# chanchanchan97/ICAFusion

Measured on AMD Instinct MI355X. Metric: RGB/IR image-pairs/sec (two-stream forward + NMS), higher is better.
Workload: dtype bf16

## Files before the change

### icafusion_amd/csrc/pool.hip

```cpp
#include "icaf_common.h"
#include <cstdlib>
#include <algorithm>
#include <cstdint>

namespace icaf {

template <int DT>
__global__ __launch_bounds__(256) void preprocess_kernel(const float* __restrict__ img, typename Elem<DT>::type* __restrict__ out,
                                                         int B, int C, int H, int W, int Cpad, int mode) {
    using E = Elem<DT>;
    const int Ho = mode ? H / 2 : H, Wo = mode ? W / 2 : W;
    const long long npix = (long long)B * Ho * Wo;
    const int nv = Cpad / E::VEC;
    for (long long pix = (long long)blockIdx.x * blockDim.x + threadIdx.x; pix < npix; pix += (long long)gridDim.x * blockDim.x) {
        const int wo = (int)(pix % Wo);
        const long long t = pix / Wo;
        const int ho = (int)(t % Ho), b = (int)(t / Ho);
        for (int v = 0; v < nv; ++v) {
            float f[E::VEC];
#pragma unroll
            for (int j = 0; j < E::VEC; ++j) {
                const int ch = v * E::VEC + j;
                float val = 0.0f;
                if (mode == 0) {
                    if (ch < C) val = img[(((long long)b * C + ch) * H + ho) * W + wo];
                } else if (ch < 4 * C) {
                    const int sub = ch / C, c = ch - sub * C, dy = sub >> 1, dx = sub & 1;
                    val = img[(((long long)b * C + c) * H + 2 * ho + dy) * W + 2 * wo + dx];
                }
                f[j] = val;
            }
            *(u32x4*)(out + pix * Cpad + v * E::VEC) = pack16<DT>(f);
        }
    }
}

template <int DT>
__global__ __launch_bounds__(256) void preprocess_u8_kernel(const unsigned char* __restrict__ img, typename Elem<DT>::type* __restrict__ out,
                                                            int B, int Ctot, int c0, int C, int nstreams, int H, int W, int Cpad, int mode) {
    using E = Elem<DT>;
    const int Ho = mode ? H / 2 : H, Wo = mode ? W / 2 : W;
    const long long npix = (long long)nstreams * B * Ho * Wo;
    const int nv = Cpad / E::VEC;
    for (long long pix = (long long)blockIdx.x * blockDim.x + threadIdx.x; pix < npix; pix += (long long)gridDim.x * blockDim.x) {
        const int wo = (int)(pix % Wo);
        long long t = pix / Wo;
        const int ho = (int)(t % Ho);
        t /= Ho;
        const int b = (int)(t % B), st = (int)(t / B);
        const unsigned char* src = img + ((long long)b * Ctot + c0 + st * C) * H * W;
        for (int v = 0; v < nv; ++v) {
            float f[E::VEC];
#pragma unroll
            for (int j = 0; j < E::VEC; ++j) {
                const int ch = v * E::VEC + j;
                float val = 0.0f;
                if (mode == 0) {
                    if (ch < C) val = (float)src[((long long)ch * H + ho) * W + wo] / 255.0f;
                } else if (ch < 4 * C) {
                    const int sub = ch / C, c = ch - sub * C, dy = sub >> 1, dx = sub & 1;
                    val = (float)src[((long long)c * H + 2 * ho + dy) * W + 2 * wo + dx] / 255.0f;
                }
                f[j] = val;
            }
            *(u32x4*)(out + pix * Cpad + v * E::VEC) = pack16<DT>(f);
        }
    }
}


template <int DT>
__global__ __launch_bounds__(256) void sppf_kernel(const typename Elem<DT>::type* __restrict__ x, int ldx,
                                                   typename Elem<DT>::type* __restrict__ y1, typename Elem<DT>::type* __restrict__ y2,
                                                   typename Elem<DT>::type* __restrict__ y3, int ldy, int B, int H, int W, int C, int k) {
    using E = Elem<DT>;
    const int nv = C / E::VEC;
    const long long total = (long long)B * H * W * nv;
    const int r1 = k / 2, r2 = 2 * r1, r3 = 3 * r1;
    for (long long idx = (long long)blockIdx.x * blockDim.x + threadIdx.x; idx < total; idx += (long long)gridDim.x * blockDim.x) {
        const int v = (int)(idx % nv);
        const long long pix = idx / nv;
        const int w = (int)(pix % W);
        const long long t = pix / W;
        const int h = (int)(t % H), b = (int)(t / H);
        float m1[E::VEC], m2[E::VEC], m3[E::VEC];
#pragma unroll
        for (int j = 0; j < E::VEC; ++j) m1[j] = m2[j] = m3[j] = -INFINITY;
        for (int dy = -r3; dy <= r3; ++dy) {
            const int hh = h + dy;
            if ((unsigned)hh >= (unsigned)H) continue;
            const int ady = dy < 0 ? -dy : dy;
            for (int dx = -r3; dx <= r3; ++dx) {
                const int ww = w + dx;
                if ((unsigned)ww >= (unsigned)W) continue;
                const int adx = dx < 0 ? -dx : dx;
                const int rad = ady > adx ? ady : adx;
                float f[E::VEC];
                unpack16<DT>(*(const u32x4*)(x + (((long long)b * H + hh) * W + ww) * ldx + v * E::VEC), f);
#pragma unroll
                for (int j = 0; j < E::VEC; ++j) {
                    m3[j] = fmaxf(m3[j], f[j]);
                    if (rad <= r2) m2[j] = fmaxf(m2[j], f[j]);
                    if (rad <= r1) m1[j] = fmaxf(m1[j], f[j]);
                }
            }
        }
        const long long o = pix * ldy + v * E::VEC;
        *(u32x4*)(y1 + o) = pack16<DT>(m1);
        *(u32x4*)(y2 + o) = pack16<DT>(m2);
        *(u32x4*)(y3 + o) = pack16<DT>(m3);
    }
}


__device__ __forceinline__ unsigned int key16x2(unsigned int b) {
    const unsigned int sign = b & 0x80008000u;
    return b ^ ((sign >> 15) * 0x7fffu | 0x80008000u);
}
__device__ __forceinline__ u32x4 key_vec(u32x4 v) { return u32x4{key16x2(v[0]), key16x2(v[1]), key16x2(v[2]), key16x2(v[3])}; }
__device__ __forceinline__ unsigned int unkey16x2(unsigned int k) {
    const unsigned int pos = k & 0x80008000u;
    return k ^ (((pos ^ 0x80008000u) >> 15) * 0x7fffu | 0x80008000u);
}
__device__ __forceinline__ u32x4 unkey_vec(u32x4 v) { return u32x4{unkey16x2(v[0]), unkey16x2(v[1]), unkey16x2(v[2]), unkey16x2(v[3])}; }
__device__ __forceinline__ unsigned int max_u16x2(unsigned int a, unsigned int b) {
    using u16x2 = __attribute__((ext_vector_type(2))) unsigned short;
    const u16x2 x = __builtin_bit_cast(u16x2, a), y = __builtin_bit_cast(u16x2, b);
    const u16x2 m = __builtin_elementwise_max(x, y);
    return __builtin_bit_cast(unsigned int, m);
}

template <int DT> struct PlaneMax {
    static __device__ __forceinline__ u32x4 in(u32x4 v) { return key_vec(v); }
    static __device__ __forceinline__ u32x4 out(u32x4 v) { return unkey_vec(v); }
    static __device__ __forceinline__ u32x4 mx(u32x4 a, u32x4 b) {
        return u32x4{max_u16x2(a[0], b[0]), max_u16x2(a[1], b[1]), max_u16x2(a[2], b[2]), max_u16x2(a[3], b[3])};
    }
};
template <> struct PlaneMax<ICAF_F32> {
    static __device__ __forceinline__ u32x4 in(u32x4 v) { return v; }
    static __device__ __forceinline__ u32x4 out(u32x4 v) { return v; }
    static __device__ __forceinline__ u32x4 mx(u32x4 a, u32x4 b) {
        u32x4 r;
#pragma unroll
        for (int j = 0; j < 4; ++j) r[j] = __float_as_uint(fmaxf(__uint_as_float(a[j]), __uint_as_float(b[j])));
        return r;
    }
};

template <int DT>
__global__ __launch_bounds__(256) void sppf_lds_kernel(const typename Elem<DT>::type* __restrict__ x, int ldx,
                                                       typename Elem<DT>::type* __restrict__ y1, typename Elem<DT>::type* __restrict__ y2,
                                                       typename Elem<DT>::type* __restrict__ y3, int ldy, int H, int W, int C, int k,
                                                       int vpb) {
    using E = Elem<DT>;
    using PM = PlaneMax<DT>;
    extern __shared__ __attribute__((aligned(16))) unsigned char smem[];
    u32x4* cur = (u32x4*)smem;
    u32x4* tmp = cur + (size_t)H * W * vpb;
    const int nvb = (C / E::VEC) / vpb;
    const int b = blockIdx.x / nvb, vg = blockIdx.x - b * nvb;
    const int n = H * W * vpb, r = k / 2;
    const long long pix0 = (long long)b * H * W;
    constexpr int MAXIT = 8;
    short iv[MAXIT], ix[MAXIT], iy[MAXIT];
#pragma unroll
    for (int t = 0; t < MAXIT; ++t) {
        const int i = threadIdx.x + t * 256;
        const int ii = i < n ? i : 0;
        const int v = ii % vpb, pp = ii / vpb;
        iv[t] = (short)v; ix[t] = (short)(pp % W); iy[t] = (short)(pp / W);
    }
#pragma unroll
    for (int t = 0; t < MAXIT; ++t) {
        const int i = threadIdx.x + t * 256;
        if (i < n) cur[i] = PM::in(*(const u32x4*)(x + (pix0 + iy[t] * W + ix[t]) * ldx + (vg * vpb + iv[t]) * E::VEC));
    }
    __syncthreads();
    typename E::type* outs[3] = {y1, y2, y3};
#pragma unroll
    for (int stage = 0; stage < 3; ++stage) {
#pragma unroll
        for (int t = 0; t < MAXIT; ++t) {
            const int i = threadIdx.x + t * 256;
            if (i >= n) continue;
            const int xx = ix[t];
            u32x4 m = cur[i];
            for (int d = -r; d <= r; ++d) {
                if (d == 0 || (unsigned)(xx + d) >= (unsigned)W) continue;
                m = PM::mx(m, cur[i + d * vpb]);
            }
            tmp[i] = m;
        }
        __syncthreads();
#pragma unroll
        for (int t = 0; t < MAXIT; ++t) {
            const int i = threadIdx.x + t * 256;
            if (i >= n) continue;
            const int yy = iy[t];
            u32x4 m = tmp[i];
            for (int d = -r; d <= r; ++d) {
                if (d == 0 || (unsigned)(yy + d) >= (unsigned)H) continue;
                m = PM::mx(m, tmp[i + d * W * vpb]);
            }
            cur[i] = m;
            *(u32x4*)(outs[stage] + (pix0 + yy * W + ix[t]) * ldy + (vg * vpb + iv[t]) * E::VEC) = PM::out(m);
        }
        __syncthreads();
    }
}

struct PoolDiv { FastDiv nv, wo, ho; };

template <int DT, bool I32>
__global__ __launch_bounds__(256) void maxpool_kernel(const typename Elem<DT>::type* __restrict__ x, int ldx, typename Elem<DT>::type* __restrict__ y,
                                                      int ldy, int B, int H, int W, int Ho, int Wo, int nv, int k, int st, int pad, PoolDiv dv) {
    using E = Elem<DT>;
    const long long total = (long long)B * Ho * Wo * nv;
    for (long long idx = (long long)blockIdx.x * blockDim.x + threadIdx.x; idx < total; idx += (long long)gridDim.x * blockDim.x) {
        long long pix;
        int v, wo, ho, b;
        if constexpr (I32) {
            unsigned int upix, uv, t, uwo, ub, uho;
            fd_divmod((unsigned int)idx, dv.nv, upix, uv);
            fd_divmod(upix, dv.wo, t, uwo);
            fd_divmod(t, dv.ho, ub, uho);
            pix = upix; v = (int)uv; wo = (int)uwo; ho = (int)uho; b = (int)ub;
        } else {
            v = (int)(idx % nv);
            pix = idx / nv;
            wo = (int)(pix % Wo);
            const long long t = pix / Wo;
            ho = (int)(t % Ho);
            b = (int)(t / Ho);
        }
        float m[E::VEC];
#pragma unroll
        for (int j = 0; j < E::VEC; ++j) m[j] = -INFINITY;
        const int h0 = ho * st - pad, w0 = wo * st - pad;
        for (int dy = 0; dy < k; ++dy) {
            const int hh = h0 + dy;
            if ((unsigned)hh >= (unsigned)H) continue;
            for (int dx = 0; dx < k; ++dx) {
                const int ww = w0 + dx;
                if ((unsigned)ww >= (unsigned)W) continue;
                float f[E::VEC];
                unpack16<DT>(*(const u32x4*)(x + (((long long)b * H + hh) * W + ww) * ldx + v * E::VEC), f);
#pragma unroll
                for (int j = 0; j < E::VEC; ++j) m[j] = (f[j] > m[j] || f[j] != f[j]) ? f[j] : m[j];
            }
        }
        *(u32x4*)(y + pix * ldy + v * E::VEC) = pack16<DT>(m);
    }
}

template <int DT>
__global__ __launch_bounds__(256) void maxpool_scalar_kernel(const typename Elem<DT>::type* __restrict__ x, int ldx, typename Elem<DT>::type* __restrict__ y,
                                                             int ldy, int B, int H, int W, int Ho, int Wo, int C, int k, int st, int pad) {
    using E = Elem<DT>;
    const long long total = (long long)B * Ho * Wo * C;
    for (long long idx = (long long)blockIdx.x * blockDim.x + threadIdx.x; idx < total; idx += (long long)gridDim.x * blockDim.x) {
        const int c = (int)(idx % C);
        const long long pix = idx / C;
        const int wo = (int)(pix % Wo);
        const long long t = pix / Wo;
        const int ho = (int)(t % Ho), b = (int)(t / Ho);
        float m = -INFINITY;
        const int h0 = ho * st - pad, w0 = wo * st - pad;
        for (int dy = 0; dy < k; ++dy) {
            const int hh = h0 + dy;
            if ((unsigned)hh >= (unsigned)H) continue;
            for (int dx = 0; dx < k; ++dx) {
                const int ww = w0 + dx;
                if ((unsigned)ww >= (unsigned)W) continue;
                const float f = E::ld(x + (((long long)b * H + hh) * W + ww) * ldx + c);
                m = (f > m || f != f) ? f : m;
            }
        }
        E::st(y + pix * ldy + c, m);
    }
}

struct UpsampleDiv { FastDiv nv, wo, ho, scale; };

template <bool I32>
__global__ __launch_bounds__(256) void upsample_kernel(const u32x4* __restrict__ x, int ldxv, u32x4* __restrict__ y, int ldyv,
                                                       int B, int H, int W, int nv, int scale, UpsampleDiv dv) {
    const int Ho = H * scale, Wo = W * scale;
    const long long total = (long long)B * Ho * Wo * nv;
    for (long long idx = (long long)blockIdx.x * blockDim.x + threadIdx.x; idx < total; idx += (long long)gridDim.x * blockDim.x) {
        if constexpr (I32) {
            unsigned int pix, v, t, wo, b, ho;
            fd_divmod((unsigned int)idx, dv.nv, pix, v);
            fd_divmod(pix, dv.wo, t, wo);
            fd_divmod(t, dv.ho, b, ho);
            const unsigned int hi = fd_div(ho, dv.scale), wi = fd_div(wo, dv.scale);
            y[(long long)pix * ldyv + v] = x[(((long long)b * H + hi) * W + wi) * ldxv + v];
        } else {
            const int v = (int)(idx % nv);
            const long long pix = idx / nv;
            const int wo = (int)(pix % Wo);
            const long long t = pix / Wo;
            const int ho = (int)(t % Ho), b = (int)(t / Ho);
            y[pix * ldyv + v] = x[(((long long)b * H + ho / scale) * W + wo / scale) * ldxv + v];
        }
    }
}

__global__ __launch_bounds__(256) void copy_kernel(const u32x4* __restrict__ x, int ldxv, u32x4* __restrict__ y, int ldyv,
                                                   long long rows, int nv) {
    const long long total = rows * nv;
    for (long long idx = (long long)blockIdx.x * blockDim.x + threadIdx.x; idx < total; idx += (long long)gridDim.x * blockDim.x) {
        const int v = (int)(idx % nv);
        const long long r = idx / nv;
        y[r * ldyv + v] = x[r * ldxv + v];
    }
}

template <int DT>
__global__ __launch_bounds__(256) void axpby_kernel(const typename Elem<DT>::type* __restrict__ x0, int ld0,
                                                    const typename Elem<DT>::type* __restrict__ x1, int ld1,
                                                    typename Elem<DT>::type* __restrict__ y, int ldy, long long rows, int nv, float a, float b) {
    using E = Elem<DT>;
    const long long total = rows * nv;
    for (long long idx = (long long)blockIdx.x * blockDim.x + threadIdx.x; idx < total; idx += (long long)gridDim.x * blockDim.x) {
        const int v = (int)(idx % nv);
        const long long r = idx / nv;
        float f0[E::VEC], f1[E::VEC], o[E::VEC];
        unpack16<DT>(*(const u32x4*)(x0 + r * ld0 + v * E::VEC), f0);
        unpack16<DT>(*(const u32x4*)(x1 + r * ld1 + v * E::VEC), f1);
#pragma unroll
        for (int j = 0; j < E::VEC; ++j) o[j] = f0[j] * a + f1[j] * b;
        *(u32x4*)(y + r * ldy + v * E::VEC) = pack16<DT>(o);
    }
}

static inline unsigned grid_for(long long total) {
    long long b = (total + 255) / 256;
    if (b > 256 * 16) b = 256 * 16;
    if (b < 1) b = 1;
    return (unsigned)b;
}

static inline int vec_of(int dtype) { return dtype == ICAF_F32 ? 4 : 8; }

}

using namespace icaf;

extern "C" int icaf_preprocess_nchw(const float* img, void* out, int dtype, int B, int C, int H, int W, int Cpad, int mode,
                                    icaf_stream_t s) {
    if (!img || !out) return fail(ICAF_ERR_ARG, "icaf_preprocess_nchw: null pointer");
    if (dtype < 0 || dtype > 2) return fail(ICAF_ERR_ARG, "icaf_preprocess_nchw: bad dtype");
    const int vec = vec_of(dtype);
    if (Cpad % vec) return fail(ICAF_ERR_ARG, "icaf_preprocess_nchw: Cpad %d must be a multiple of %d", Cpad, vec);
    if (mode == 1 && ((H | W) & 1)) return fail(ICAF_ERR_ARG, "icaf_preprocess_nchw: space-to-depth needs even H, W");
    if (mode == 1 ? Cpad < 4 * C : Cpad < C) return fail(ICAF_ERR_ARG, "icaf_preprocess_nchw: Cpad too small");
    const long long total = (long long)B * (mode ? H / 2 : H) * (mode ? W / 2 : W);
    dim3 grid(grid_for(total)), block(256);
    if (dtype == ICAF_F32) hipLaunchKernelGGL(preprocess_kernel<ICAF_F32>, grid, block, 0, S(s), img, (float*)out, B, C, H, W, Cpad, mode);
    else if (dtype == ICAF_BF16) hipLaunchKernelGGL(preprocess_kernel<ICAF_BF16>, grid, block, 0, S(s), img, (unsigned short*)out, B, C, H, W, Cpad, mode);
    else hipLaunchKernelGGL(preprocess_kernel<ICAF_F16>, grid, block, 0, S(s), img, (unsigned short*)out, B, C, H, W, Cpad, mode);
    ICAF_LAUNCH_CHECK();
    return ICAF_OK;
}

extern "C" int icaf_preprocess_u8(const unsigned char* img, void* out, int dtype, int B, int Ctot, int c0, int C, int nstreams, int H,
                                  int W, int Cpad, int mode, icaf_stream_t s) {
    if (!img || !out) return fail(ICAF_ERR_ARG, "icaf_preprocess_u8: null pointer");
    if (dtype < 0 || dtype > 2) return fail(ICAF_ERR_ARG, "icaf_preprocess_u8: bad dtype");
    const int vec = vec_of(dtype);
    if (Cpad % vec) return fail(ICAF_ERR_ARG, "icaf_preprocess_u8: Cpad %d must be a multiple of %d", Cpad, vec);
    if (mode == 1 && ((H | W) & 1)) return fail(ICAF_ERR_ARG, "icaf_preprocess_u8: space-to-depth needs even H, W");
    if (mode == 1 ? Cpad < 4 * C : Cpad < C) return fail(ICAF_ERR_ARG, "icaf_preprocess_u8: Cpad too small");
    if (nstreams < 1 || c0 < 0 || c0 + nstreams * C > Ctot) return fail(ICAF_ERR_ARG, "icaf_preprocess_u8: channels [%d, %d) exceed %d", c0, c0 + nstreams * C, Ctot);
    const long long total = (long long)nstreams * B * (mode ? H / 2 : H) * (mode ? W / 2 : W);
    dim3 grid(grid_for(total)), block(256);
    if (dtype == ICAF_F32) hipLaunchKernelGGL(preprocess_u8_kernel<ICAF_F32>, grid, block, 0, S(s), img, (float*)out, B, Ctot, c0, C, nstreams, H, W, Cpad, mode);
    else if (dtype == ICAF_BF16) hipLaunchKernelGGL(preprocess_u8_kernel<ICAF_BF16>, grid, block, 0, S(s), img, (unsigned short*)out, B, Ctot, c0, C, nstreams, H, W, Cpad, mode);
    else hipLaunchKernelGGL(preprocess_u8_kernel<ICAF_F16>, grid, block, 0, S(s), img, (unsigned short*)out, B, Ctot, c0, C, nstreams, H, W, Cpad, mode);
    ICAF_LAUNCH_CHECK();
    return ICAF_OK;
}


static int sppf_select(int dtype, int H, int W, int C) {
    const int nv = C / vec_of(dtype);
    int cap = 8;
    if (g_opt.sppf_vpb > 0) cap = g_opt.sppf_vpb;
    for (int c : {8, 4, 2, 1})
        if (c <= cap && nv % c == 0 && (size_t)H * W * c * 32 <= 60 * 1024) return c;
    return 0;
}

extern "C" int icaf_sppf_config(int dtype, int H, int W, int C, int* vpb) {
    if (!vpb) return fail(ICAF_ERR_ARG, "icaf_sppf_config: null pointer");
    if (dtype < 0 || dtype > 2) return fail(ICAF_ERR_ARG, "icaf_sppf_config: bad dtype");
    if (H < 1 || W < 1 || C < 1 || C % vec_of(dtype)) return fail(ICAF_ERR_ARG, "icaf_sppf_config: bad geometry");
    *vpb = sppf_select(dtype, H, W, C);
    return ICAF_OK;
}

extern "C" int icaf_sppf_pool(const void* x, int ldx, void* y1, void* y2, void* y3, int ldy, int dtype, int B, int H, int W, int C,
                              int k, icaf_stream_t s) {
    if (!x || !y1 || !y2 || !y3) return fail(ICAF_ERR_ARG, "icaf_sppf_pool: null pointer");
    if (dtype < 0 || dtype > 2) return fail(ICAF_ERR_ARG, "icaf_sppf_pool: bad dtype");
    const int vec = vec_of(dtype);
    if (C % vec || ldx % vec || ldy % vec || !(k & 1)) return fail(ICAF_ERR_ARG, "icaf_sppf_pool: C/ld must be multiples of %d and k odd", vec);
    const int nv = C / vec;
    const int vpb = sppf_select(dtype, H, W, C);
    if (vpb) {
        const size_t lds = (size_t)H * W * vpb * 32;
        dim3 grid((unsigned)(B * (nv / vpb))), block(256);
        if (dtype == ICAF_F32) sppf_lds_kernel<ICAF_F32><<<grid, block, lds, S(s)>>>((const float*)x, ldx, (float*)y1, (float*)y2, (float*)y3, ldy, H, W, C, k, vpb);
        else if (dtype == ICAF_BF16) sppf_lds_kernel<ICAF_BF16><<<grid, block, lds, S(s)>>>((const unsigned short*)x, ldx, (unsigned short*)y1, (unsigned short*)y2, (unsigned short*)y3, ldy, H, W, C, k, vpb);
        else sppf_lds_kernel<ICAF_F16><<<grid, block, lds, S(s)>>>((const unsigned short*)x, ldx, (unsigned short*)y1, (unsigned short*)y2, (unsigned short*)y3, ldy, H, W, C, k, vpb);
        ICAF_LAUNCH_CHECK();
        return ICAF_OK;
    }
    const long long total = (long long)B * H * W * (C / vec);
    dim3 grid(grid_for(total)), block(256);
    if (dtype == ICAF_F32) hipLaunchKernelGGL(sppf_kernel<ICAF_F32>, grid, block, 0, S(s), (const float*)x, ldx, (float*)y1, (float*)y2, (float*)y3, ldy, B, H, W, C, k);
    else if (dtype == ICAF_BF16) hipLaunchKernelGGL(sppf_kernel<ICAF_BF16>, grid, block, 0, S(s), (const unsigned short*)x, ldx, (unsigned short*)y1, (unsigned short*)y2, (unsigned short*)y3, ldy, B, H, W, C, k);
    else hipLaunchKernelGGL(sppf_kernel<ICAF_F16>, grid, block, 0, S(s), (const unsigned short*)x, ldx, (unsigned short*)y1, (unsigned short*)y2, (unsigned short*)y3, ldy, B, H, W, C, k);
    ICAF_LAUNCH_CHECK();
    return ICAF_OK;
}

extern "C" int icaf_upsample_nearest(const void* x, int ldx, void* y, int ldy, int dtype, int B, int H, int W, int C, int scale,
                                     icaf_stream_t s) {
    if (!x || !y) return fail(ICAF_ERR_ARG, "icaf_upsample_nearest: null pointer");
    if (dtype < 0 || dtype > 2) return fail(ICAF_ERR_ARG, "icaf_upsample_nearest: bad dtype");
    const int vec = vec_of(dtype);
    if (C % vec || ldx % vec || ldy % vec || scale < 1) return fail(ICAF_ERR_ARG, "icaf_upsample_nearest: bad geometry");
    const long long total = (long long)B * H * scale * W * scale * (C / vec);
    if (total < 1) return fail(ICAF_ERR_ARG, "icaf_upsample_nearest: empty tensor");
    const UpsampleDiv dv{make_fastdiv((unsigned)(C / vec)), make_fastdiv((unsigned)(W * scale)), make_fastdiv((unsigned)(H * scale)),
                         make_fastdiv((unsigned)scale)};
    if (total < (1ll << 31) && !g_opt.index64)
        hipLaunchKernelGGL(upsample_kernel<true>, dim3(grid_for(total)), dim3(256), 0, S(s), (const u32x4*)x, ldx / vec, (u32x4*)y,
                           ldy / vec, B, H, W, C / vec, scale, dv);
    else
        hipLaunchKernelGGL(upsample_kernel<false>, dim3(grid_for(total)), dim3(256), 0, S(s), (const u32x4*)x, ldx / vec, (u32x4*)y,
                           ldy / vec, B, H, W, C / vec, scale, dv);
    ICAF_LAUNCH_CHECK();
    return ICAF_OK;
}

extern "C" int icaf_axpby(const void* x0, int ld0, const void* x1, int ld1, void* y, int ldy, int dtype, long long rows, int C, float a,
                          float b, icaf_stream_t s) {
    if (!x0 || !x1 || !y) return fail(ICAF_ERR_ARG, "icaf_axpby: null pointer");
    if (dtype < 0 || dtype > 2) return fail(ICAF_ERR_ARG, "icaf_axpby: bad dtype");
    const int vec = vec_of(dtype);
    if (C % vec || ld0 % vec || ld1 % vec || ldy % vec) return fail(ICAF_ERR_ARG, "icaf_axpby: C/ld must be multiples of %d", vec);
    dim3 grid(grid_for(rows * (C / vec))), block(256);
    if (dtype == ICAF_F32) axpby_kernel<ICAF_F32><<<grid, block, 0, S(s)>>>((const float*)x0, ld0, (const float*)x1, ld1, (float*)y, ldy, rows, C / vec, a, b);
    else if (dtype == ICAF_BF16) axpby_kernel<ICAF_BF16><<<grid, block, 0, S(s)>>>((const unsigned short*)x0, ld0, (const unsigned short*)x1, ld1, (unsigned short*)y, ldy, rows, C / vec, a, b);
    else axpby_kernel<ICAF_F16><<<grid, block, 0, S(s)>>>((const unsigned short*)x0, ld0, (const unsigned short*)x1, ld1, (unsigned short*)y, ldy, rows, C / vec, a, b);
    ICAF_LAUNCH_CHECK();
    return ICAF_OK;
}

extern "C" int icaf_copy_channels(const void* x, int ldx, void* y, int ldy, int dtype, long long rows, int C, icaf_stream_t s) {
    if (!x || !y) return fail(ICAF_ERR_ARG, "icaf_copy_channels: null pointer");
    if (dtype < 0 || dtype > 2) return fail(ICAF_ERR_ARG, "icaf_copy_channels: bad dtype");
    const int vec = vec_of(dtype);
    if (C % vec || ldx % vec || ldy % vec) return fail(ICAF_ERR_ARG, "icaf_copy_channels: C/ld must be multiples of %d", vec);
    hipLaunchKernelGGL(copy_kernel, dim3(grid_for(rows * (C / vec))), dim3(256), 0, S(s), (const u32x4*)x, ldx / vec, (u32x4*)y, ldy / vec,
                       rows, C / vec);
    ICAF_LAUNCH_CHECK();
    return ICAF_OK;
}

template <int DT>
static int launch_maxpool(const void* x, int ldx, void* y, int ldy, int B, int H, int W, int Ho, int Wo, int C, int k, int st, int pad, bool vec16,
                          hipStream_t s) {
    using T = typename Elem<DT>::type;
    constexpr int vec = Elem<DT>::VEC;
    if (!vec16) {
        const long long total = (long long)B * Ho * Wo * C;
        hipLaunchKernelGGL(maxpool_scalar_kernel<DT>, dim3(grid_for(total)), dim3(256), 0, s, (const T*)x, ldx, (T*)y, ldy, B, H, W, Ho, Wo, C, k, st, pad);
    } else {
        const int nv = C / vec;
        const long long total = (long long)B * Ho * Wo * nv;
        const PoolDiv dv{make_fastdiv((unsigned)nv), make_fastdiv((unsigned)Wo), make_fastdiv((unsigned)Ho)};
        if (total < (1ll << 31))
            hipLaunchKernelGGL((maxpool_kernel<DT, true>), dim3(grid_for(total)), dim3(256), 0, s, (const T*)x, ldx, (T*)y, ldy, B, H, W, Ho, Wo, nv, k, st, pad, dv);
        else
            hipLaunchKernelGGL((maxpool_kernel<DT, false>), dim3(grid_for(total)), dim3(256), 0, s, (const T*)x, ldx, (T*)y, ldy, B, H, W, Ho, Wo, nv, k, st, pad, dv);
    }
    ICAF_LAUNCH_CHECK();
    return ICAF_OK;
}

extern "C" int icaf_maxpool2d(const void* x, int ldx, void* y, int ldy, int dtype, int B, int H, int W, int C, int k, int stride, int pad,
                              icaf_stream_t s) {
    if (!x || !y) return fail(ICAF_ERR_ARG, "icaf_maxpool2d: null pointer");
    if (dtype < 0 || dtype > 2) return fail(ICAF_ERR_ARG, "icaf_maxpool2d: bad dtype");
    if (!((k == 2 && stride == 2 && pad == 0) || (k == 3 && stride == 2 && pad == 1)))
        return fail(ICAF_ERR_UNSUPPORTED, "icaf_maxpool2d: window (k, s, p) = (%d, %d, %d) is not built: (2, 2, 0) and (3, 2, 1) are", k, stride, pad);
    const int vec = vec_of(dtype), eb = dtype == ICAF_F32 ? 4 : 2;
    if (B < 1 || H < 1 || W < 1 || C < 1 || H + 2 * pad < k || W + 2 * pad < k) return fail(ICAF_ERR_ARG, "icaf_maxpool2d: bad geometry %d x %d x %d x %d", B, H, W, C);
    if (C % vec) return fail(ICAF_ERR_ARG, "icaf_maxpool2d: C (%d) must be a multiple of %d", C, vec);
    if (ldx < C || ldy < C) return fail(ICAF_ERR_ARG, "icaf_maxpool2d: ldx (%d) / ldy (%d) < C (%d)", ldx, ldy, C);
    if (((uintptr_t)x | (uintptr_t)y) & (uintptr_t)(eb - 1)) return fail(ICAF_ERR_ARG, "icaf_maxpool2d: x / y must be aligned to the element size");
    const int Ho = (H + 2 * pad - k) / stride + 1, Wo = (W + 2 * pad - k) / stride + 1;
    if ((long long)B * H * W > 0x7fffffffLL) return fail(ICAF_ERR_ARG, "icaf_maxpool2d: too many pixels");
    const bool vec16 = ldx % vec == 0 && ldy % vec == 0 && (((uintptr_t)x | (uintptr_t)y) & 15) == 0;
    if (dtype == ICAF_F32) return launch_maxpool<ICAF_F32>(x, ldx, y, ldy, B, H, W, Ho, Wo, C, k, stride, pad, vec16, S(s));
    if (dtype == ICAF_BF16) return launch_maxpool<ICAF_BF16>(x, ldx, y, ldy, B, H, W, Ho, Wo, C, k, stride, pad, vec16, S(s));
    return launch_maxpool<ICAF_F16>(x, ldx, y, ldy, B, H, W, Ho, Wo, C, k, stride, pad, vec16, S(s));
}
```

Before: 16630.

## Widen SPPF LDS kernel to 1024 threads and make upsample iterate over input pixels

The SPPF LDS kernel moves to 1024-thread blocks with two items per thread. It precomputes global offsets, adds a k=5 specialised path that clamps neighbour indices so loads are unconditional, and swaps __syncthreads for a lighter LDS-wait barrier. The aim is shorter serial loops per thread and more memory-level parallelism. Nearest upsample now runs one thread per input element that writes all scale×scale outputs, with two elements in flight per iteration, which cuts index division and redundant input reads. The larger blocks may limit occupancy, and the static_assert ties correctness to plane sizes of at most 60×1024/32 items.

```diff
diff --git a/icafusion_amd/csrc/pool.hip b/icafusion_amd/csrc/pool.hip
--- a/icafusion_amd/csrc/pool.hip
+++ b/icafusion_amd/csrc/pool.hip
@@ -148,11 +148,44 @@
     }
 };
 
+__device__ __forceinline__ void plane_barrier() {
+    asm volatile("s_waitcnt lgkmcnt(0)" ::: "memory");
+    __builtin_amdgcn_s_barrier();
+    asm volatile("" ::: "memory");
+}
+
+constexpr int SPPF_THREADS = 1024;
+constexpr int SPPF_MAXIT = 2;
+static_assert(SPPF_THREADS * SPPF_MAXIT >= 60 * 1024 / 32, "every item of the largest plane needs a thread");
+
+template <int DT, int R>
+__device__ __forceinline__ void sppf_pass_fixed(const u32x4* __restrict__ src, const int* li, const short* pos, int len, int step, u32x4* m) {
+    using PM = PlaneMax<DT>;
+    u32x4 nb[SPPF_MAXIT][2 * R];
+#pragma unroll
+    for (int t = 0; t < SPPF_MAXIT; ++t) {
+        const int p = pos[t];
+        m[t] = src[li[t]];
+#pragma unroll
+        for (int d = -R, j = 0; d <= R; ++d) {
+            if (d == 0) continue;
+            const int q = min(max(p + d, 0), len - 1);
+            nb[t][j++] = src[li[t] + (q - p) * step];
+        }
+    }
+#pragma unroll
+    for (int t = 0; t < SPPF_MAXIT; ++t)
+#pragma unroll
+        for (int j = 0; j < 2 * R; ++j) m[t] = PM::mx(m[t], nb[t][j]);
+#pragma unroll
+    for (int t = 0; t < SPPF_MAXIT; ++t) asm volatile("" : "+v"(m[t]));
+}
+
 template <int DT>
-__global__ __launch_bounds__(256) void sppf_lds_kernel(const typename Elem<DT>::type* __restrict__ x, int ldx,
-                                                       typename Elem<DT>::type* __restrict__ y1, typename Elem<DT>::type* __restrict__ y2,
-                                                       typename Elem<DT>::type* __restrict__ y3, int ldy, int H, int W, int C, int k,
-                                                       int vpb) {
+__global__ __launch_bounds__(SPPF_THREADS) void sppf_lds_kernel(const typename Elem<DT>::type* __restrict__ x, int ldx,
+                                                                typename Elem<DT>::type* __restrict__ y1, typename Elem<DT>::type* __restrict__ y2,
+                                                                typename Elem<DT>::type* __restrict__ y3, int ldy, int H, int W, int C, int k,
+                                                                int vpb) {
     using E = Elem<DT>;
     using PM = PlaneMax<DT>;
     extern __shared__ __attribute__((aligned(16))) unsigned char smem[];
@@ -162,28 +195,57 @@
     const int b = blockIdx.x / nvb, vg = blockIdx.x - b * nvb;
     const int n = H * W * vpb, r = k / 2;
     const long long pix0 = (long long)b * H * W;
-    constexpr int MAXIT = 8;
-    short iv[MAXIT], ix[MAXIT], iy[MAXIT];
+    constexpr int MAXIT = SPPF_MAXIT;
+    short ix[MAXIT], iy[MAXIT];
+    int li[MAXIT];
+    bool has[MAXIT];
+    long long gx[MAXIT], gy[MAXIT];
 #pragma unroll
     for (int t = 0; t < MAXIT; ++t) {
-        const int i = threadIdx.x + t * 256;
-        const int ii = i < n ? i : 0;
-        const int v = ii % vpb, pp = ii / vpb;
-        iv[t] = (short)v; ix[t] = (short)(pp % W); iy[t] = (short)(pp / W);
-    }
-#pragma unroll
-    for (int t = 0; t < MAXIT; ++t) {
-        const int i = threadIdx.x + t * 256;
-        if (i < n) cur[i] = PM::in(*(const u32x4*)(x + (pix0 + iy[t] * W + ix[t]) * ldx + (vg * vpb + iv[t]) * E::VEC));
-    }
-    __syncthreads();
+        const int i = threadIdx.x + t * SPPF_THREADS;
+        has[t] = i < n;
+        li[t] = has[t] ? i : 0;
+        const int v = li[t] % vpb, pp = li[t] / vpb;
+        ix[t] = (short)(pp % W); iy[t] = (short)(pp / W);
+        gx[t] = (pix0 + pp) * ldx + (vg * vpb + v) * E::VEC;
+        gy[t] = (pix0 + pp) * ldy + (vg * vpb + v) * E::VEC;
+    }
+    u32x4 in[MAXIT];
+#pragma unroll
+    for (int t = 0; t < MAXIT; ++t) in[t] = *(const u32x4*)(x + gx[t]);
+#pragma unroll
+    for (int t = 0; t < MAXIT; ++t) asm volatile("" : "+v"(in[t]));
+#pragma unroll
+    for (int t = 0; t < MAXIT; ++t)
+        if (has[t]) cur[li[t]] = PM::in(in[t]);
+    plane_barrier();
     typename E::type* outs[3] = {y1, y2, y3};
+    if (k == 5) {
+#pragma unroll
+        for (int stage = 0; stage < 3; ++stage) {
+            u32x4 m[MAXIT];
+            sppf_pass_fixed<DT, 2>(cur, li, ix, W, vpb, m);
+#pragma unroll
+            for (int t = 0; t < MAXIT; ++t)
+                if (has[t]) tmp[li[t]] = m[t];
+            plane_barrier();
+            sppf_pass_fixed<DT, 2>(tmp, li, iy, H, W * vpb, m);
+#pragma unroll
+            for (int t = 0; t < MAXIT; ++t)
+                if (has[t]) {
+                    if (stage < 2) cur[li[t]] = m[t];
+                    *(u32x4*)(outs[stage] + gy[t]) = PM::out(m[t]);
+                }
+            if (stage < 2) plane_barrier();
+        }
+        return;
+    }
 #pragma unroll
     for (int stage = 0; stage < 3; ++stage) {
 #pragma unroll
         for (int t = 0; t < MAXIT; ++t) {
-            const int i = threadIdx.x + t * 256;
-            if (i >= n) continue;
+            const int i = li[t];
+            if (!has[t]) continue;
             const int xx = ix[t];
             u32x4 m = cur[i];
             for (int d = -r; d <= r; ++d) {
@@ -192,11 +254,11 @@
             }
             tmp[i] = m;
         }
-        __syncthreads();
+        plane_barrier();
 #pragma unroll
         for (int t = 0; t < MAXIT; ++t) {
-            const int i = threadIdx.x + t * 256;
-            if (i >= n) continue;
+            const int i = li[t];
+            if (!has[t]) continue;
             const int yy = iy[t];
             u32x4 m = tmp[i];
             for (int d = -r; d <= r; ++d) {
@@ -204,9 +266,9 @@
                 m = PM::mx(m, tmp[i + d * W * vpb]);
             }
             cur[i] = m;
-            *(u32x4*)(outs[stage] + (pix0 + yy * W + ix[t]) * ldy + (vg * vpb + iv[t]) * E::VEC) = PM::out(m);
-        }
-        __syncthreads();
+            *(u32x4*)(outs[stage] + gy[t]) = PM::out(m);
+        }
+        plane_barrier();
     }
 }
 
@@ -281,29 +343,64 @@
     }
 }
 
-struct UpsampleDiv { FastDiv nv, wo, ho, scale; };
+struct UpsampleDiv { FastDiv nv, w; };
+
+template <bool I32>
+__device__ __forceinline__ void upsample_where(long long idx, int ldxv, int ldyv, int W, int nv, int scale, const UpsampleDiv& dv,
+                                               long long& xo, long long& yo) {
+    long long pix, bh;
+    int v, wi;
+    if constexpr (I32) {
+        unsigned int upix, uv, ubh, uwi;
+        fd_divmod((unsigned int)idx, dv.nv, upix, uv);
+        fd_divmod(upix, dv.w, ubh, uwi);
+        pix = upix; v = (int)uv; bh = ubh; wi = (int)uwi;
+    } else {
+        v = (int)(idx % nv);
+        pix = idx / nv;
+        wi = (int)(pix % W);
+        bh = pix / W;
+    }
+    xo = pix * ldxv + v;
+    yo = ((bh * scale) * ((long long)W * scale) + (long long)wi * scale) * ldyv + v;
+}
+
+__device__ __forceinline__ void upsample_store(u32x4* __restrict__ y, long long yo, long long rowv, int ldyv, int scale, u32x4 val) {
+    if (scale == 2) {
+        y[yo] = val;
+        y[yo + ldyv] = val;
+        y[yo + rowv] = val;
+        y[yo + rowv + ldyv] = val;
+        return;
+    }
+    for (int dy = 0; dy < scale; ++dy)
+        for (int dx = 0; dx < scale; ++dx) y[yo + dy * rowv + (long long)dx * ldyv] = val;
+}
 
 template <bool I32>
 __global__ __launch_bounds__(256) void upsample_kernel(const u32x4* __restrict__ x, int ldxv, u32x4* __restrict__ y, int ldyv,
                                                        int B, int H, int W, int nv, int scale, UpsampleDiv dv) {
-    const int Ho = H * scale, Wo = W * scale;
-    const long long total = (long long)B * Ho * Wo * nv;
-    for (long long idx = (long long)blockIdx.x * blockDim.x + threadIdx.x; idx < total; idx += (long long)gridDim.x * blockDim.x) {
-        if constexpr (I32) {
-            unsigned int pix, v, t, wo, b, ho;
-            fd_divmod((unsigned int)idx, dv.nv, pix, v);
-            fd_divmod(pix, dv.wo, t, wo);
-            fd_divmod(t, dv.ho, b, ho);
-            const unsigned int hi = fd_div(ho, dv.scale), wi = fd_div(wo, dv.scale);
-            y[(long long)pix * ldyv + v] = x[(((long long)b * H + hi) * W + wi) * ldxv + v];
-        } else {
-            const int v = (int)(idx % nv);
-            const long long pix = idx / nv;
-            const int wo = (int)(pix % Wo);
-            const long long t = pix / Wo;
-            const int ho = (int)(t % Ho), b = (int)(t / Ho);
-            y[pix * ldyv + v] = x[(((long long)b * H + ho / scale) * W + wo / scale) * ldxv + v];
-        }
+    const long long total = (long long)B * H * W * nv;
+    const long long stride = (long long)gridDim.x * blockDim.x;
+    const long long rowv = (long long)W * scale * ldyv;
+    const long long first = (long long)blockIdx.x * blockDim.x + threadIdx.x;
+    if (total <= stride) {
+        if (first < total) {
+            long long xo, yo;
+            upsample_where<I32>(first, ldxv, ldyv, W, nv, scale, dv, xo, yo);
+            upsample_store(y, yo, rowv, ldyv, scale, x[xo]);
+        }
+        return;
+    }
+    for (long long idx = first; idx < total; idx += 2 * stride) {
+        const bool two = idx + stride < total;
+        long long xo0, yo0, xo1, yo1;
+        upsample_where<I32>(idx, ldxv, ldyv, W, nv, scale, dv, xo0, yo0);
+        upsample_where<I32>(two ? idx + stride : idx, ldxv, ldyv, W, nv, scale, dv, xo1, yo1);
+        u32x4 a = x[xo0], b = x[xo1];
+        asm volatile("" : "+v"(a), "+v"(b));
+        upsample_store(y, yo0, rowv, ldyv, scale, a);
+        if (two) upsample_store(y, yo1, rowv, ldyv, scale, b);
     }
 }
 
@@ -411,7 +508,7 @@
     const int vpb = sppf_select(dtype, H, W, C);
     if (vpb) {
         const size_t lds = (size_t)H * W * vpb * 32;
-        dim3 grid((unsigned)(B * (nv / vpb))), block(256);
+        dim3 grid((unsigned)(B * (nv / vpb))), block(SPPF_THREADS);
         if (dtype == ICAF_F32) sppf_lds_kernel<ICAF_F32><<<grid, block, lds, S(s)>>>((const float*)x, ldx, (float*)y1, (float*)y2, (float*)y3, ldy, H, W, C, k, vpb);
         else if (dtype == ICAF_BF16) sppf_lds_kernel<ICAF_BF16><<<grid, block, lds, S(s)>>>((const unsigned short*)x, ldx, (unsigned short*)y1, (unsigned short*)y2, (unsigned short*)y3, ldy, H, W, C, k, vpb);
         else sppf_lds_kernel<ICAF_F16><<<grid, block, lds, S(s)>>>((const unsigned short*)x, ldx, (unsigned short*)y1, (unsigned short*)y2, (unsigned short*)y3, ldy, H, W, C, k, vpb);
@@ -435,13 +532,13 @@
     if (C % vec || ldx % vec || ldy % vec || scale < 1) return fail(ICAF_ERR_ARG, "icaf_upsample_nearest: bad geometry");
     const long long total = (long long)B * H * scale * W * scale * (C / vec);
     if (total < 1) return fail(ICAF_ERR_ARG, "icaf_upsample_nearest: empty tensor");
-    const UpsampleDiv dv{make_fastdiv((unsigned)(C / vec)), make_fastdiv((unsigned)(W * scale)), make_fastdiv((unsigned)(H * scale)),
-                         make_fastdiv((unsigned)scale)};
+    const UpsampleDiv dv{make_fastdiv((unsigned)(C / vec)), make_fastdiv((unsigned)W)};
+    const dim3 grid(grid_for((long long)B * H * W * (C / vec)));
     if (total < (1ll << 31) && !g_opt.index64)
-        hipLaunchKernelGGL(upsample_kernel<true>, dim3(grid_for(total)), dim3(256), 0, S(s), (const u32x4*)x, ldx / vec, (u32x4*)y,
+        hipLaunchKernelGGL(upsample_kernel<true>, grid, dim3(256), 0, S(s), (const u32x4*)x, ldx / vec, (u32x4*)y,
                            ldy / vec, B, H, W, C / vec, scale, dv);
     else
-        hipLaunchKernelGGL(upsample_kernel<false>, dim3(grid_for(total)), dim3(256), 0, S(s), (const u32x4*)x, ldx / vec, (u32x4*)y,
+        hipLaunchKernelGGL(upsample_kernel<false>, grid, dim3(256), 0, S(s), (const u32x4*)x, ldx / vec, (u32x4*)y,
                            ldy / vec, B, H, W, C / vec, scale, dv);
     ICAF_LAUNCH_CHECK();
     return ICAF_OK;
```

Result: no change. 16560 (-0.4%).
